# Gardlin/PCR-CG

Measured on AMD Instinct MI355X. Metric: fragment-pairs/s KPFCNN+GCN fwd, 30k-pt pairs, higher is better.
Workload: dtype f32

## Files before the change

include/pcrcg.h:

```cpp
#ifndef PCRCG_H
#define PCRCG_H

#include <stddef.h>
#include <stdint.h>

#ifdef __cplusplus
extern "C" {
#endif

#define PCRCG_OK 0
#define PCRCG_EBADARG (-1)
#define PCRCG_EWORKSPACE (-2)
#define PCRCG_ELAUNCH (-3)
#define PCRCG_ECAPACITY (-4)

#define PCRCG_KPOINTS 15

const char* pcrcg_last_error(void);
#define PCRCG_ABI_VERSION 4
int pcrcg_abi_version(void);

int pcrcg_debug_set(const char* spec);
int pcrcg_debug_release(void);

// ... 47 lines not shown
                         const void* forest, int cloud0, float radius, const int* rows, int nrows, const int* count,
                         int max_count, int cols, int64_t* idx, int* status, void* stream);
int pcrcg_radius_reorder_jobs(const pcrcg_reorder_job* jobs, int njobs, const float* sup, int ns, int nb,
                              const void* forest, int* status, void* stream);

size_t pcrcg_kpconv_ws_bytes(int ns);
int pcrcg_kpconv_aggregate(const float* q_pts, int nq, const float* s_pts, int ns, const int64_t* idx,
                           int h, int ld_idx, const float* x, int cin, const float* kp, float extent,
                           float* wf, float* inv_n, void* ws, size_t ws_bytes, void* stream);
int pcrcg_kpconv_aggregate_bf16(const float* q_pts, int nq, const float* s_pts, int ns, const int64_t* idx, int h,
                                int ld_idx, const float* x, int cin, const float* kp, float extent, void* x_bf16,
                                void* wf_bf16, float* inv_n, void* ws, size_t ws_bytes, void* stream);

void pcrcg_profile_kpconv(int enable);
int pcrcg_profile_kpconv_read(float* ms, int* nq, int* h, int* cin, int* cout, int* kind, int cap);

int pcrcg_gemm_f32(const float* a, int lda, const float* b, int ldb, int trans_b, float* c, int ldc, int m,
                   int n, int k, const float* row_scale, const float* bias, void* stream);
size_t pcrcg_gemm_colstats_bytes(int m, int n);
int pcrcg_gemm_f32_colstats(const float* a, int lda, const float* b, int ldb, int trans_b, float* c, int ldc,
                            int m, int n, int k, const float* row_scale, const float* bias, void* colstats,
                            size_t colstats_bytes, int* h_chunks, void* stream);
int pcrcg_gemm_bf16a_f32_colstats(const void* a_bf16, int lda, const float* b, int ldb, float* c, int ldc, int m, int n,
                                  int k, const float* row_scale, const float* bias, void* colstats,
                                  size_t colstats_bytes, int* h_chunks, void* stream);

int pcrcg_gemm_f32_fused(const float* a, int lda, const int64_t* idx, int ld_idx, int ns, const float* zero_row,
                         const void* a_sums, double a_count, float a_eps, float a_slope, const float* b, int ldb,
                         const float* bias, float* c, int ldc, int m, int n, int k, int accumulate, void* stream);

void pcrcg_gemm_set_mode(int mode);
int pcrcg_gemm_get_mode(void);
int pcrcg_gemm_redo_counts(unsigned long long* out2, int reset);
void pcrcg_thread_shares_gpu(int on);

int pcrcg_gather_max(const float* x, int ns, int c, const int64_t* idx, int nq, int h, int ld_idx,
                     float* out, void* stream);
int pcrcg_gather_first(const float* x, int ns, int c, const int64_t* idx, int nq, int ld_idx, float* out,
                       int ld_out, void* stream);
size_t pcrcg_instnorm_ws_bytes(int c);
int pcrcg_instnorm_stats_from_partials(const void* partials, int chunks, int c, double count, float eps,
                                       float* stats, void* stream);
int pcrcg_instnorm_stats(const float* x, int n, int c, int ldx, float eps, float* stats, void* ws,
                         size_t ws_bytes, void* stream);
int pcrcg_instnorm_apply(const float* x, int n, int c, int ldx, const float* stats, const float* res,
                         int ldr, const float* res_stats, float slope, float* y, int ldy, void* stream);
int pcrcg_instnorm_colsums(const float* x, int n, int c, int ldx, void* sums, void* stream);
int pcrcg_instnorm_apply_sums(const float* x, int n, int c, int ldx, const void* sums, double count, float eps,
                              const float* res, int ldr, const void* res_sums, float slope, float* y, int ldy,
                              void* stream);

int pcrcg_fill2d(float* dst, int ld, int rows, int cols, float value, void* stream);
int pcrcg_inject_image_features(const float* fmap, int c, int h, int w, const float* valid, const int64_t* inds2d,
                                const int64_t* inds3d, int n, long row_offset, long n_rows, float* x, int ldx,
                                void* stream);

typedef struct pcrcg_image_frame {
    const float* fmap;
    const float* depth;
    const float* valid;
    float world2camera[16];
    float intrinsics[16];
    float thresh;
    int h, w;
    int depth_h, depth_w;
    int target;
// ... 190 lines not shown
```

pcrcg_amd/_lib.py:

```python
import ctypes
import os

_HERE = os.path.dirname(os.path.abspath(__file__))
LIB_PATH = os.path.join(_HERE, "libpcrcg_hip.so")


def lib_identity():
    import hashlib
    with open(LIB_PATH, "rb") as f:
        return LIB_PATH, hashlib.sha256(f.read()).hexdigest()[:16]

ABI_VERSION = 4

c_int, c_float, c_void_p, c_size_t = ctypes.c_int, ctypes.c_float, ctypes.c_void_p, ctypes.c_size_t

SIGNATURES = {
    "pcrcg_last_error": (ctypes.c_char_p, []),
    "pcrcg_abi_version": (c_int, []),
    "pcrcg_debug_set": (c_int, [ctypes.c_char_p]),
    "pcrcg_check_status": (c_int, [c_void_p, c_void_p]),
    "pcrcg_grid_subsample_ws_bytes": (c_size_t, [c_int, c_int]),
    "pcrcg_grid_subsample_batch": (c_int, [c_void_p, c_int, c_void_p, c_int, c_float, c_int, c_void_p, c_void_p,
                                           c_void_p, c_void_p, c_size_t, c_void_p]),
    "pcrcg_umap_order_ws_bytes": (c_size_t, [c_int]),
# ... 7 lines not shown
    "pcrcg_radius_query_groups": (c_int, [c_void_p, c_int, c_void_p, c_int, c_void_p, c_int, c_int, c_float, c_void_p, c_int,
                                          c_void_p, c_void_p, c_void_p, c_void_p, c_void_p, c_void_p, c_void_p]),
    "pcrcg_radius_query_cells": (c_int, [c_void_p, c_void_p, c_int, c_void_p, c_void_p, c_int, c_void_p, c_int, c_int, c_float,
                                         c_int, c_void_p, c_void_p, c_void_p, c_void_p, c_void_p, c_void_p, c_void_p]),
    "pcrcg_kdforest_ws_bytes": (c_size_t, [c_int, c_int]),
    "pcrcg_kdforest_build": (c_int, [c_void_p, c_int, c_void_p, c_int, c_void_p, c_size_t, c_void_p]),
    "pcrcg_radius_reorder": (c_int, [c_void_p, c_int, c_void_p, c_int, c_void_p, c_int, c_int, c_void_p, c_int,
                                     c_float, c_void_p, c_int, c_void_p, c_int, c_int, c_void_p, c_void_p, c_void_p]),
    "pcrcg_radius_reorder_jobs": (c_int, [c_void_p, c_int, c_void_p, c_int, c_int, c_void_p, c_void_p, c_void_p]),
    "pcrcg_radius_neighbors_ws_bytes": (c_size_t, [c_int, c_int]),
    "pcrcg_radius_neighbors_batch": (c_int, [c_void_p, c_int, c_void_p, c_int, c_void_p, c_void_p, c_int, c_float,
                                             c_int, c_void_p, c_void_p, c_void_p, c_void_p, c_void_p, c_size_t,
                                             c_void_p]),
    "pcrcg_kpconv_ws_bytes": (c_size_t, [c_int]),
    "pcrcg_kpconv_aggregate": (c_int, [c_void_p, c_int, c_void_p, c_int, c_void_p, c_int, c_int, c_void_p, c_int,
                                       c_void_p, c_float, c_void_p, c_void_p, c_void_p, c_size_t, c_void_p]),
    "pcrcg_kpconv_aggregate_bf16": (c_int, [c_void_p, c_int, c_void_p, c_int, c_void_p, c_int, c_int, c_void_p, c_int,
                                            c_void_p, c_float, c_void_p, c_void_p, c_void_p, c_void_p, c_size_t,
                                            c_void_p]),
    "pcrcg_profile_kpconv": (None, [c_int]),
    "pcrcg_profile_kpconv_read": (c_int, [c_void_p, c_void_p, c_void_p, c_void_p, c_void_p, c_void_p, c_int]),
    "pcrcg_gemm_f32": (c_int, [c_void_p, c_int, c_void_p, c_int, c_int, c_void_p, c_int, c_int, c_int, c_int,
                               c_void_p, c_void_p, c_void_p]),
    "pcrcg_gemm_colstats_bytes": (c_size_t, [c_int, c_int]),
    "pcrcg_gemm_f32_colstats": (c_int, [c_void_p, c_int, c_void_p, c_int, c_int, c_void_p, c_int, c_int, c_int, c_int,
                                        c_void_p, c_void_p, c_void_p, c_size_t, c_void_p, c_void_p]),
    "pcrcg_gemm_bf16a_f32_colstats": (c_int, [c_void_p, c_int, c_void_p, c_int, c_void_p, c_int, c_int, c_int, c_int,
                                              c_void_p, c_void_p, c_void_p, c_size_t, c_void_p, c_void_p]),
    "pcrcg_gemm_f32_fused": (c_int, [c_void_p, c_int, c_void_p, c_int, c_int, c_void_p, c_void_p, ctypes.c_double, c_float,
                                     c_float, c_void_p, c_int, c_void_p, c_void_p, c_int, c_int, c_int, c_int, c_int, c_void_p]),
    "pcrcg_gemm_set_mode": (None, [c_int]),
    "pcrcg_gemm_get_mode": (c_int, []),
    "pcrcg_gemm_redo_counts": (c_int, [c_void_p, c_int]),
    "pcrcg_instnorm_stats_from_partials": (c_int, [c_void_p, c_int, c_int, ctypes.c_double, c_float, c_void_p,
                                                   c_void_p]),
    "pcrcg_gather_max": (c_int, [c_void_p, c_int, c_int, c_void_p, c_int, c_int, c_int, c_void_p, c_void_p]),
    "pcrcg_gather_first": (c_int, [c_void_p, c_int, c_int, c_void_p, c_int, c_int, c_void_p, c_int, c_void_p]),
    "pcrcg_instnorm_ws_bytes": (c_size_t, [c_int]),
    "pcrcg_instnorm_stats": (c_int, [c_void_p, c_int, c_int, c_int, c_float, c_void_p, c_void_p, c_size_t, c_void_p]),
    "pcrcg_instnorm_apply": (c_int, [c_void_p, c_int, c_int, c_int, c_void_p, c_void_p, c_int, c_void_p, c_float,
                                     c_void_p, c_int, c_void_p]),
    "pcrcg_instnorm_colsums": (c_int, [c_void_p, c_int, c_int, c_int, c_void_p, c_void_p]),
    "pcrcg_instnorm_apply_sums": (c_int, [c_void_p, c_int, c_int, c_int, c_void_p, ctypes.c_double, c_float, c_void_p, c_int,
                                          c_void_p, c_float, c_void_p, c_int, c_void_p]),
    "pcrcg_fill2d": (c_int, [c_void_p, c_int, c_int, c_int, c_float, c_void_p]),
    "pcrcg_inject_image_features": (c_int, [c_void_p, c_int, c_int, c_int, c_void_p, c_void_p, c_void_p, c_int, ctypes.c_long,
                                            ctypes.c_long, c_void_p, c_int, c_void_p]),
    "pcrcg_project_depth_ws_bytes": (c_size_t, [c_int]),
    "pcrcg_project_depth": (c_int, [c_void_p, c_int, c_void_p, c_int, c_int, c_void_p, c_void_p, c_float, c_void_p, c_void_p,
                                    c_void_p, c_void_p, c_size_t, c_void_p]),
    "pcrcg_inject_frames": (c_int, [c_void_p, ctypes.c_long, ctypes.c_long, c_void_p, c_int, c_int, c_void_p, c_int, c_void_p]),
    "pcrcg_superglue_valid_maps": (c_int, [c_void_p, c_int, c_void_p, c_int, c_void_p, c_void_p, c_int, c_int, c_int, c_void_p,
                                           c_void_p, c_void_p]),
    "pcrcg_knn": (c_int, [c_void_p, c_int, c_int, c_void_p, c_void_p]),
    "pcrcg_edgeconv_ws_bytes": (c_size_t, [c_int]),
    "pcrcg_edgeconv_reduce": (c_int, [c_void_p, c_int, c_void_p, c_int, c_void_p, c_int, c_int, c_int, c_float,
                                      c_void_p, c_int, c_void_p, c_void_p, c_size_t, c_void_p]),
    "pcrcg_edgeconv_reduce_sums": (c_int, [c_void_p, c_int, c_void_p, c_int, c_void_p, c_int, c_int, c_int, c_void_p, c_int,
                                           c_void_p, c_void_p]),
    "pcrcg_softmax_rows": (c_int, [c_void_p, c_int, c_int, c_int, c_float, c_void_p]),
    "pcrcg_attention_supported": (c_int, [c_int]),
    "pcrcg_attention": (c_int, [c_void_p, c_int, c_void_p, c_int, c_void_p, c_int, c_void_p, c_int, c_int, c_int, c_int,
                                c_int, c_float, c_void_p]),
    "pcrcg_softmax_matvec": (c_int, [c_void_p, c_int, c_int, c_int, c_float, c_void_p, c_int, c_void_p, c_int, c_void_p]),
    "pcrcg_copy2d": (c_int, [c_void_p, c_int, c_void_p, c_int, c_int, c_int, c_void_p]),
    "pcrcg_add": (c_int, [c_void_p, c_void_p, c_void_p, ctypes.c_long, c_void_p]),
# ... 117 lines not shown
```

pcrcg_amd/csrc/common.h:

```cpp
#pragma once
#include <hip/hip_runtime.h>

#include <cstdarg>
#include <cstdint>
#include <cstdio>
#include <mutex>

#include "pcrcg.h"

namespace pcrcg {

void set_error(const char* fmt, ...);

inline hipStream_t as_stream(void* s) { return reinterpret_cast<hipStream_t>(s); }

struct Carver {
    char* base;
    size_t cap;
    size_t off = 0;
    Carver(void* ws, size_t bytes) : base(static_cast<char*>(ws)), cap(bytes) {}
    template <typename T>
    T* take(size_t count) {
        size_t bytes = (count * sizeof(T) + 255) & ~size_t(255);
        T* p = reinterpret_cast<T*>(base + off);
// ... 87 lines not shown
int gather_max_multi(const GatherJob* jobs, int count, int c, hipStream_t st);
int heads_multi(const float* const* x, const int* rows, int count, int ld, int fd, float* const* feats, float* const* s_ov,
                float* const* s_sal, hipStream_t st);
int copy2d_multi(const float* const* src, float* const* dst, const int* rows, int count, int ld_src, int ld_dst, int cols,
                 hipStream_t st);
int instnorm_colsums_multi(const float* const* x, double* const* sums, const int* n, int count, int c, int ldx, hipStream_t st);

struct EdgeCloud {
    const float* ctr; const float* nbr; const int* idx; float* emax; double* sums; int n, k;
};
bool edgeconv_rows_ok(const EdgeCloud* cl, int count, int ld_ctr, int ld_nbr, int ld_emax, int c);
int edgeconv_rows_multi(const EdgeCloud* cl, int count, int ld_ctr, int ld_nbr, int ld_emax, int c, bool atomic, int* nchunks_out,
                        hipStream_t st);

struct AttnCloud { const float* q; const float* k; const float* v; float* out; int n, ms; };
bool attention_mfma_ok(const AttnCloud* cl, int count, int ldq, int ldk, int ldv, int d);
int attention_mfma_multi(const AttnCloud* cl, int count, int ldq, int ldk, int ldv, int ldo, int heads, int d, float scale,
                         hipStream_t st);
bool attention_bwd_mfma_ok(int n, int ms, int d, int ldq, int ldk, int ldv, int ld_do);
int attention_bwd_mfma(const float* q, int ldq, const float* k, int ldk, const float* v, int ldv, const float* o, int ldo,
                       const float* d_o, int ld_do, float* dq, int ld_dq, float* dk, int ld_dk, float* dv, int ld_dv, int n, int ms,
                       int heads, int d, float scale, hipStream_t st);

struct DebugOpts {
    int stat_sums = 1;
    int stat_sums_rows = 1 << 30;
    int att_mfma = 1;
    int radius_blocks = 0;
    int kd_blocks = 0;
    int att_tq = 16;
    int kd_spin_limit = 0;
    int gemm_log = 0;
    int x6_tile = -1, x6_splitk = 0, x6_t1 = 1, x6_t2 = 1, x6_order = -1, x6_big = 0, x6_h2 = 1;
    int train_side_stream = 1;
    int gemm_tile = -1, gemm_splitk = 0, gemm_split_target = 768;
    int deterministic = 0;
    int bwd_mfma = 1;
};
const DebugOpts& debug_opts();

struct KpProfScope {
    hipStream_t st;
    hipEvent_t a, b;
    int nq, h, cin, cout, kind;
    bool on;
    KpProfScope(hipStream_t s, int nq, int h, int cin, int cout, int kind);
    ~KpProfScope();
};

}

#define PCRCG_CHECK_ARG(cond)                                                        \
    do {                                                                             \
        if (!(cond)) {                                                               \
            pcrcg::set_error("%s: bad argument: %s", __func__, #cond);               \
            return PCRCG_EBADARG;                                                    \
        }                                                                            \
    } while (0)

#define PCRCG_CHECK_WS(carver)                                                                     \
    do {                                                                                           \
        if (!(carver).ok()) {                                                                      \
            pcrcg::set_error("%s: workspace too small (%zu needed, %zu given)", __func__,          \
                             (carver).off, (carver).cap);                                          \
            return PCRCG_EWORKSPACE;                                                               \
        }                                                                                          \
// ... 36 lines not shown
```

pcrcg_amd/csrc/gemm.hip:

```cpp
#include <cstdlib>

#include <atomic>

#include "common.h"
#include "pcrcg_train.h"

namespace pcrcg {
namespace {

typedef float f32x16 __attribute__((ext_vector_type(16)));
template <int BM, int BN, bool TRANS_A, bool TRANS_B, int BK>
constexpr int stage_floats() {
    return (TRANS_A ? BK * (BM + 4) : BM * (BK + 4)) + (TRANS_B ? BN * (BK + 4) : BK * (BN + 4));
}

template <int BM, int BN, int WAVES_M, int WAVES_N, bool TRANS_A, bool TRANS_B, int BK>
__global__ void __launch_bounds__(256) k_gemm_f32(const float* __restrict__ A, int lda, const float* __restrict__ B,
                                                   int ldb, float* __restrict__ C, int ldc, int M, int N, int Kdim,
                                                   const float* __restrict__ row_scale, const float* __restrict__ bias,
                                                   int k_per_split, int vec_a, int vec_b, int atomic_out,
                                                   double* __restrict__ colp, int colp_chunks) {
    static_assert(WAVES_M * WAVES_N == 4, "4 wavefronts per block");
    constexpr int WM = BM / WAVES_M, WN = BN / WAVES_N;
    constexpr int TM = WM / 32, TN = WN / 32;
// ... 272 lines not shown
                                                          k_per_split, vec_a, vec_b, atomic_out, colp, colp_chunks);
    return launch_one<BM, BN, WAVES_M, WAVES_N, false, false, BK>(grid, st, a, lda, b, ldb, c, ldc, m, n, k, row_scale, bias,
                                                       k_per_split, vec_a, vec_b, atomic_out, colp, colp_chunks);
}

}
}

namespace pcrcg {
int gemm_x6_dispatch(const float* a, int lda, const float* b, int ldb, float* c, int ldc, int m, int n, int k,
                     const float* row_scale, const float* bias, void* colstats, size_t colstats_bytes, int* h_chunks,
                     hipStream_t st, bool a_bf16, bool c_zeroed, int a_kmajor = 0, int b_kmajor = 0,
                     bool colstats_sums = false, const GemmExtra* ex = nullptr, const GemmGroup* grp = nullptr);
int gemm_x6_splits(int m, int n, int k, long m_total = 0);
}

using namespace pcrcg;

static std::atomic<int> g_gemm_mode{-1};
static int gemm_mode() {
    int mode = g_gemm_mode.load(std::memory_order_relaxed);
    if (mode < 0) {
        const char* e = getenv("PCRCG_GEMM_MODE");
        int want = e ? (atoi(e) != 0) : 1, expect = -1;
        g_gemm_mode.compare_exchange_strong(expect, want, std::memory_order_relaxed);
        mode = g_gemm_mode.load(std::memory_order_relaxed);
    }
    return mode;
}
extern "C" void pcrcg_gemm_set_mode(int mode) { g_gemm_mode.store(mode != 0, std::memory_order_relaxed); }
extern "C" void pcrcg_thread_shares_gpu(int on) { gemm_x6_set_shared(on); }
namespace pcrcg { int gemm_x6_redo_counts(unsigned long long* out, int reset); }
extern "C" int pcrcg_gemm_redo_counts(unsigned long long* out2, int reset) { return gemm_x6_redo_counts(out2, reset); }
extern "C" int pcrcg_gemm_get_mode(void) { return gemm_mode(); }

static int gemm_dispatch(const float* a, int lda, int trans_a, const float* b, int ldb, int trans_b, float* c, int ldc,
                         int m, int n, int k, const float* row_scale, const float* bias, void* colstats,
                         size_t colstats_bytes, int* h_chunks, void* stream, bool c_zeroed = false,
                         bool colstats_sums = false);

namespace pcrcg {
bool gemm_bt_accumulates(int m, int n, int k, long m_total) { return gemm_mode() == 1 && gemm_x6_splits(m, n, k, m_total) > 1; }
bool gemm_colstats_sums_ok() { return gemm_mode() == 1; }
bool gemm_extra_ok() { return gemm_mode() == 1; }
int gemm_bt_extra(const float* a, int lda, const float* b, int ldb, float* c, int ldc, int m, int n, int k, hipStream_t st,
                  bool c_zeroed, const GemmExtra& ex, const float* bias, void* colstats, size_t colstats_bytes, int* h_chunks,
                  bool colstats_sums) {
    if (h_chunks) *h_chunks = 0;
    PCRCG_CHECK_ARG(m >= 0 && n >= 0 && k >= 1 && lda >= k && ldb >= k && ldc >= n);
    if (m == 0 || n == 0) return PCRCG_OK;
    PCRCG_CHECK_ARG(a && b && c && gemm_mode() == 1);
    return gemm_x6_dispatch(a, lda, b, ldb, c, ldc, m, n, k, nullptr, bias, colstats, colstats_bytes, h_chunks, st, false,
                            c_zeroed, 0, 0, colstats_sums, &ex);
}
bool gemm_pair_ok() { return gemm_mode() == 1; }
int gemm_bt_colstats_pair(const float* a, int lda, const float* b, int ldb, float* c, int ldc, int m, int n, int k,
                          const float* row_scale, const float* bias, void* colstats, size_t colstats_bytes, int* h_chunks,
                          hipStream_t st, bool c_zeroed, bool colstats_sums, const GemmGroup* pair) {
    if (!pair || pair->n == 0)
        return gemm_dispatch(a, lda, 0, b, ldb, 1, c, ldc, m, n, k, row_scale, bias, colstats, colstats_bytes, h_chunks, st,
                             c_zeroed, colstats_sums);
    if (h_chunks) *h_chunks = 0;
    PCRCG_CHECK_ARG(m >= 1 && n >= 1 && k >= 1 && lda >= k && ldb >= k && ldc >= n);
    PCRCG_CHECK_ARG(a && b && c && gemm_mode() == 1);
    return gemm_x6_dispatch(a, lda, b, ldb, c, ldc, m, n, k, row_scale, bias, colstats, colstats_bytes, h_chunks, st, false,
                            c_zeroed, 0, 0, colstats_sums, nullptr, pair);
// ... 184 lines not shown
```

pcrcg_amd/csrc/gemm_x6.hip:

```cpp
#include <cstdlib>
#include <map>
#include <mutex>
#include <type_traits>

#include <hip/hip_ext.h>

#include "common.h"
#include "pcrcg_train.h"

namespace pcrcg {
namespace {

typedef float f32x16 __attribute__((ext_vector_type(16)));
typedef __bf16 bf16x8 __attribute__((ext_vector_type(8)));
typedef unsigned int u32x4 __attribute__((ext_vector_type(4)));

typedef float f32x4 __attribute__((ext_vector_type(4)));
typedef float f32x2 __attribute__((ext_vector_type(2)));
typedef _Float16 f16x2 __attribute__((ext_vector_type(2)));
typedef _Float16 f16x8 __attribute__((ext_vector_type(8)));

constexpr int BK = 32;

__device__ unsigned long long g_x6_redo[2];

constexpr int kGroupExtra = 3;
struct GemmPairArgs {
    int extra = 0;
    int off[kGroupExtra] = {0, 0, 0}, m[kGroupExtra] = {0, 0, 0};
    const float* a[kGroupExtra] = {nullptr, nullptr, nullptr};
    float* c[kGroupExtra] = {nullptr, nullptr, nullptr};
    const float* rs[kGroupExtra] = {nullptr, nullptr, nullptr};
// ... 662 lines not shown
        double* const red = reinterpret_cast<double*>(smem);
        __syncthreads();
#pragma unroll
        for (int j = 0; j < TN; ++j) {
            const double s = ds[j] + __shfl_xor(ds[j], 32, 64), q2 = dq[j] + __shfl_xor(dq[j], 32, 64);
            if (wm == 1 && half == 0) {
                red[2 * (wn * WN + j * 32 + l31)] = s;
                red[2 * (wn * WN + j * 32 + l31) + 1] = q2;
            }
        }
        __syncthreads();
#pragma unroll
        for (int j = 0; j < TN; ++j) {
            const double s = ds[j] + __shfl_xor(ds[j], 32, 64), q2 = dq[j] + __shfl_xor(dq[j], 32, 64);
            const int gn = n0 + wn * WN + j * 32 + l31;
            if (wm == 0 && half == 0 && gn < N) {
                unsafeAtomicAdd(&colp[gn], s + red[2 * (wn * WN + j * 32 + l31)]);
                unsafeAtomicAdd(&colp[(long)N + gn], q2 + red[2 * (wn * WN + j * 32 + l31) + 1]);
            }
        }
    } else if (colp) {
        const int chunk = tile_y * WAVES_M + wm;
#pragma unroll
        for (int j = 0; j < TN; ++j) {
            const double s = ds[j] + __shfl_xor(ds[j], 32, 64), q2 = dq[j] + __shfl_xor(dq[j], 32, 64);
            const int gn = n0 + wn * WN + j * 32 + l31;
            if (half == 0 && gn < N) {
                colp[(long)gn * colp_chunks + chunk] = s;
                colp[((long)N + gn) * colp_chunks + chunk] = q2;
            }
        }
    }
}

thread_local long g_split_stride = 0;
thread_local bool g_det_pass = false;
struct DetBuf { float* p = nullptr; size_t n = 0; };
std::mutex g_det_mu;
std::map<hipStream_t, DetBuf> g_det_bufs;
float* det_partials(hipStream_t st, size_t floats) {
    std::lock_guard<std::mutex> g(g_det_mu);
    DetBuf& b = g_det_bufs[st];
    if (b.n < floats) {
        if (hipStreamSynchronize(st) != hipSuccess) return nullptr;
        if (b.p) (void)hipFree(b.p);
        b.p = nullptr;
        b.n = 0;
        const size_t want = floats + floats / 4;
        if (hipMalloc(&b.p, want * sizeof(float)) != hipSuccess) { b.p = nullptr; return nullptr; }
        b.n = want;
    }
    return b.p;
}

__global__ void __launch_bounds__(256) k_split_reduce(const float* __restrict__ part, long stride, int splits, float* __restrict__ c,
                                                      int ldc, int m, int n, int accumulate) {
    const long t = (long)blockIdx.x * 256 + threadIdx.x;
    if (t >= (long)m * n) return;
    const long r = t / n;
    const int col = (int)(t - r * n);
    float sum = part[t];
    for (int s = 1; s < splits; ++s) sum += part[(long)s * stride + t];
    float* dst = c + r * ldc + col;
    *dst = accumulate ? *dst + sum : sum;
}

template <int BM, int BN, int MINB, int ATERMS, int ALAY, int BLAY, int ANORM = 0, int KNOCK = 0, int H2 = 0>
int launch_x6(dim3 grid, hipStream_t st, const float* a, int lda, const float* b, int ldb, float* c, int ldc, int m, int n,
              int k, const float* row_scale, const float* bias, int k_per_split, int vec_a, int vec_b, int atomic_out,
              double* colp, int colp_chunks, const long long* a_idx = nullptr, int a_idx_ld = 0, int a_ns = 0,
              const float* a_zero = nullptr, const double* a_sums = nullptr, double a_count = 0.0, float a_eps = 0.f,
              float a_slope = 1.f, GemmPairArgs pr = GemmPairArgs(), float h2_sa = 1.f, float h2_sb = 1.f) {
    TileMap tm;
    tm.split_stride = g_split_stride;
    tm.gx = (int)grid.x;
    tm.gy = (int)grid.y;
    tm.gs = (int)grid.z;
    tm.order = x6_tile_order(tm.gx, tm.gy, tm.gs, BM, BN, k_per_split);
    const size_t lds = lds_bytes<BM, BN>() + (ANORM ? 2 * sizeof(float) * (size_t)(((k_per_split + BK - 1) / BK) * BK) : 0) + (H2 ? 16 : 0);
    auto kern = k_gemm_x6<BM, BN, MINB, ATERMS, ALAY, BLAY, ANORM, KNOCK, H2>;
    PCRCG_GRANT_LDS(kern);
    int m_all = m;
    for (int e = 0; e < pr.extra; ++e) m_all += pr.m[e];
    KpProfScope prof(st, m_all, n, k, (ATERMS == 1 || H2) ? 3 : 6, 3);
    hipExtLaunchKernelGGL(kern, dim3(tm.gx * tm.gy * tm.gs), dim3(x6_threads<BM, BN>()), lds, st, prof.a, prof.b, 0, a, lda, b, ldb, c, ldc, m, n,
                          k, row_scale, bias, k_per_split, vec_a, vec_b, atomic_out, colp, colp_chunks, a_idx, a_idx_ld, a_ns,
                          a_zero, a_sums, a_count, a_eps, a_slope, pr, tm, h2_sa, h2_sb);
    PCRCG_CHECK_LAUNCH();
    return PCRCG_OK;
}


}

static thread_local int g_x6_shared = 0;
bool gemm_x6_shared() { return g_x6_shared > 0; }
void gemm_x6_set_shared(int on) { g_x6_shared = on ? 1 : 0; }

struct X6Plan { int pick, bm, bn, gx, gy, splits, k_per_split; };
static X6Plan x6_plan_for(int pick, int m, int n, int k, bool reduce_rows) {
    static const int tiles[4][2] = {{128, 128}, {128, 64}, {64, 128}, {64, 64}};
    X6Plan p;
    p.pick = pick;
    p.bm = tiles[p.pick][0];
    p.bn = tiles[p.pick][1];
    p.gx = (n + p.bn - 1) / p.bn;
    p.gy = (m + p.bm - 1) / p.bm;
    int splits = 1;
    const int ktiles = (k + BK - 1) / BK;
    const int max_splits = reduce_rows ? 128 : 32;
    int t1 = 200, t2 = 1024;
    if (gemm_x6_shared() && !reduce_rows) { t1 = debug_opts().x6_t1; t2 = debug_opts().x6_t2; }
    while ((long)p.gx * p.gy * splits < t1 && k / (2 * splits) >= 256 && splits < max_splits) splits *= 2;
    while ((long)p.gx * p.gy * splits < t2 && k / splits > 1024 && splits < max_splits) splits *= 2;
    if (debug_opts().x6_splitk > 0) splits = debug_opts().x6_splitk;
    p.k_per_split = ((ktiles + splits - 1) / splits) * BK;
    if (p.k_per_split < BK) p.k_per_split = BK;
    p.splits = k > 0 ? (k + p.k_per_split - 1) / p.k_per_split : 1;
    if (p.splits < 1) p.splits = 1;
    return p;
}
static X6Plan x6_plan(int m, int n, int k, bool kmajor = false, bool reduce_rows = false, long m_total = 0) {
    int pick = debug_opts().x6_tile;
    if (kmajor) return x6_plan_for(3, m, n, k, reduce_rows);
    if (pick >= 0 && pick <= 3) return x6_plan_for(pick, m, n, k, reduce_rows);
    if (n >= 128 && debug_opts().x6_big) {
        const X6Plan big = x6_plan_for(0, m, n, k, reduce_rows);
        const long rows = m_total > m ? m_total : m;
        if ((long)big.gx * ((rows + 127) / 128) * big.splits >= 240) return big;
    }
    return x6_plan_for((n <= 64 && m >= 32768) ? 1 : 3, m, n, k, reduce_rows);
}

int gemm_x6_redo_counts(unsigned long long* out, int reset) {
    if (out) PCRCG_CHECK_HIP(hipMemcpyFromSymbol(out, HIP_SYMBOL(g_x6_redo), sizeof(unsigned long long) * 2));
    if (reset) {
        const unsigned long long z[2] = {0ull, 0ull};
        PCRCG_CHECK_HIP(hipMemcpyToSymbol(HIP_SYMBOL(g_x6_redo), z, sizeof(z)));
    }
    return PCRCG_OK;
}

int gemm_x6_splits(int m, int n, int k, long m_total) { return (m > 0 && n > 0) ? x6_plan(m, n, k, false, false, m_total).splits : 1; }

void gemm_x6_release_det() {
    std::lock_guard<std::mutex> g(g_det_mu);
    for (auto& kv : g_det_bufs)
        if (kv.second.p) (void)hipFree(kv.second.p);
    g_det_bufs.clear();
}

int gemm_x6_dispatch(const float* a, int lda, const float* b, int ldb, float* c, int ldc, int m, int n, int k,
                     const float* row_scale, const float* bias, void* colstats, size_t colstats_bytes, int* h_chunks,
                     hipStream_t st, bool a_bf16, bool c_zeroed, int a_kmajor, int b_kmajor, bool colstats_sums,
                     const GemmExtra* ex, const GemmGroup* grp) {
    const int vec_a = (a_bf16 || a_kmajor) ? 1 : (lda % 4 == 0) && ((reinterpret_cast<uintptr_t>(a) & 15) == 0);
    const int vec_b = b_kmajor ? 1 : (ldb % 4 == 0) && ((reinterpret_cast<uintptr_t>(b) & 15) == 0);
    if (a_kmajor && !b_kmajor) { set_error("gemm_x6: A^T * B^T is not built"); return PCRCG_EBADARG; }
    int m_plan = m;
    const int n_extra = grp ? grp->n : 0;
    if (n_extra < 0 || n_extra > kGroupExtra) { set_error("gemm_x6: at most %d further products per launch", kGroupExtra); return PCRCG_EBADARG; }
    for (int e = 0; e < n_extra; ++e) {
        if (grp->p[e].m <= 0 || !grp->p[e].a || !grp->p[e].c) { set_error("gemm_x6: empty product in a group"); return PCRCG_EBADARG; }
        m_plan = grp->p[e].m > m_plan ? grp->p[e].m : m_plan;
    }
    long m_total = m;
    for (int e = 0; e < n_extra; ++e) m_total += grp->p[e].m;
    const bool lifted = ex && ex->grad_operand && debug_opts().x6_h2 != 0 && !a_bf16;
    const X6Plan plan = x6_plan(m_plan, n, k, a_kmajor || b_kmajor || (ex && ex->a_sums) || lifted, a_kmajor != 0, m_total);
    const int pick = plan.pick, BM = plan.bm, BN = plan.bn, gx = plan.gx, splits = plan.splits;
    const int gy0 = (m + BM - 1) / BM;
    int gy = gy0, gye[kGroupExtra] = {0, 0, 0};
    for (int e = 0; e < n_extra; ++e) { gye[e] = (grp->p[e].m + BM - 1) / BM; gy += gye[e]; }
    if (n_extra && (a_kmajor || b_kmajor)) { set_error("gemm_x6: grouped launches are built for the A * B^T form"); return PCRCG_EBADARG; }
    const int k_per_split = plan.k_per_split;
// ... 28 lines not shown
                grp2.p[e].h_chunks = nullptr;
                row += (size_t)grp->p[e].m;
            }
        }
        g_det_pass = true;
        g_split_stride = (long)(rows_all * (size_t)n);
        const int rc = gemm_x6_dispatch(a, lda, b, ldb, part, n, m, n, k, row_scale, bias, nullptr, 0, nullptr, st, a_bf16, true,
                                        a_kmajor, b_kmajor, false, ex ? &ex2 : nullptr, grp ? &grp2 : nullptr);
        g_det_pass = false;
        g_split_stride = 0;
        if (rc != PCRCG_OK) return rc;
        row = 0;
        for (int e = -1; e < n_extra; ++e) {
            const int me = e < 0 ? m : grp->p[e].m;
            float* ce = e < 0 ? c : grp->p[e].c;
            const long total = (long)me * n;
            hipLaunchKernelGGL(k_split_reduce, dim3((unsigned)((total + 255) / 256)), dim3(256), 0, st, part + row * (size_t)n,
                               (long)(rows_all * (size_t)n), splits, ce, ldc, me, n, accumulate ? 1 : 0);
            row += (size_t)me;
        }
        PCRCG_CHECK_LAUNCH();
        return PCRCG_OK;
    }
    const int atomic_out = g_det_pass ? 0 : (splits > 1 || accumulate);
    if (splits > 1 && !c_zeroed && !accumulate) {
        if (ldc == n) PCRCG_CHECK_HIP(hipMemsetAsync(c, 0, (size_t)m * n * sizeof(float), st));
        else PCRCG_CHECK_HIP(hipMemset2DAsync(c, (size_t)ldc * sizeof(float), 0, (size_t)n * sizeof(float), m, st));
    }
    for (int e = 0; e < n_extra; ++e)
        if (splits > 1 && !grp->p[e].c_zeroed && !accumulate) {
            if (ldc == n) PCRCG_CHECK_HIP(hipMemsetAsync(grp->p[e].c, 0, (size_t)grp->p[e].m * n * sizeof(float), st));
            else PCRCG_CHECK_HIP(hipMemset2DAsync(grp->p[e].c, (size_t)ldc * sizeof(float), 0, (size_t)n * sizeof(float), grp->p[e].m, st));
        }
    dim3 grid(gx, gy, splits);
    const bool log_shapes = debug_opts().gemm_log != 0;
    if (log_shapes)
        fprintf(stderr, "pcrcg_gemm_x6 m=%d n=%d k=%d lda=%d ldb=%d ldc=%d tile=%dx%d grid=%dx%dx%d rs=%d bias=%d stats=%d\n", m,
                n, k, lda, ldb, ldc, BM, BN, gx, gy, splits, row_scale != nullptr, bias != nullptr, colstats != nullptr);
    double* colp = nullptr;
    int colp_chunks = 0;
    if (colstats && h_chunks && !atomic_out && colstats_sums) {
        if (2 * (size_t)n * sizeof(double) <= colstats_bytes) {
            colp = static_cast<double*>(colstats);
            colp_chunks = -1;
            *h_chunks = -1;
        }
    } else if (colstats && h_chunks && !atomic_out) {
        colp_chunks = gy0 * 2;
        if (carve_bytes(2 * (size_t)n * colp_chunks, sizeof(double)) <= colstats_bytes) {
            colp = static_cast<double*>(colstats);
            *h_chunks = colp_chunks;
        } else {
            colp_chunks = 0;
        }
    }
    GemmPairArgs pa;
    pa.extra = n_extra;
    int row_off = gy0 * BM;
    for (int e = 0; e < n_extra; ++e) {
        const GemmPair& q = grp->p[e];
        pa.off[e] = row_off;
        row_off += gye[e] * BM;
        pa.m[e] = q.m;
        pa.a[e] = q.a;
        pa.c[e] = q.c;
        pa.rs[e] = q.row_scale;
// ... 79 lines not shown
```

pcrcg_amd/csrc/scan.hip:

```cpp
#include <cstring>

#include <atomic>
#include <mutex>

#include "common.h"

namespace pcrcg {

static thread_local char g_err[512] = "";

void set_error(const char* fmt, ...) {
    va_list ap;
    va_start(ap, fmt);
    vsnprintf(g_err, sizeof(g_err), fmt, ap);
    va_end(ap);
}

namespace {

constexpr int kScanThreads = 256;
constexpr int kScanItems = 8;
constexpr int kScanTile = kScanThreads * kScanItems;

__device__ __forceinline__ int wave_inclusive_scan(int v, int lane) {
// ... 145 lines not shown
int exclusive_scan_i32(const int* in, int* out, int n, int* total, void* ws, hipStream_t stream) {
    if (n <= 0) {
        if (total) hipLaunchKernelGGL(zero_int, dim3(1), dim3(1), 0, stream, total);
        PCRCG_CHECK_LAUNCH();
        return PCRCG_OK;
    }
    const int nt = (n + kScanTile - 1) / kScanTile;
    if (nt == 1) {
        hipLaunchKernelGGL(scan_apply, dim3(1), dim3(kScanThreads), 0, stream, in, out, n,
                           (const int*)nullptr, total);
        PCRCG_CHECK_LAUNCH();
        return PCRCG_OK;
    }
    if (n <= kOneTiles * kOneThreads * kScanItems && (reinterpret_cast<uintptr_t>(in) & 15) == 0 &&
        (reinterpret_cast<uintptr_t>(out) & 15) == 0) {
        hipLaunchKernelGGL(scan_one_block, dim3(1), dim3(kOneThreads), 0, stream, in, out, n, total);
        PCRCG_CHECK_LAUNCH();
        return PCRCG_OK;
    }
    int* partial = static_cast<int*>(ws);
    hipLaunchKernelGGL(scan_tile_sums, dim3(nt), dim3(kScanThreads), 0, stream, in, n, partial);
    hipLaunchKernelGGL(scan_partials, dim3(1), dim3(kScanThreads), 0, stream, partial, nt, total);
    hipLaunchKernelGGL(scan_apply, dim3(nt), dim3(kScanThreads), 0, stream, in, out, n,
                       (const int*)partial, (int*)nullptr);
    PCRCG_CHECK_LAUNCH();
    return PCRCG_OK;
}

namespace {
struct DebugName { const char* name; int DebugOpts::*field; };
const DebugName kDebugNames[] = {
    {"stat_sums", &DebugOpts::stat_sums}, {"stat_sums_rows", &DebugOpts::stat_sums_rows}, {"att_mfma", &DebugOpts::att_mfma},
    {"radius_blocks", &DebugOpts::radius_blocks}, {"kd_blocks", &DebugOpts::kd_blocks}, {"att_tq", &DebugOpts::att_tq},
    {"kd_spin_limit", &DebugOpts::kd_spin_limit}, {"gemm_log", &DebugOpts::gemm_log}, {"x6_tile", &DebugOpts::x6_tile}, {"x6_order", &DebugOpts::x6_order}, {"x6_big", &DebugOpts::x6_big}, {"x6_h2", &DebugOpts::x6_h2}, {"train_side_stream", &DebugOpts::train_side_stream},
    {"x6_splitk", &DebugOpts::x6_splitk}, {"x6_t1", &DebugOpts::x6_t1}, {"x6_t2", &DebugOpts::x6_t2},
    {"gemm_tile", &DebugOpts::gemm_tile}, {"gemm_splitk", &DebugOpts::gemm_splitk},
    {"gemm_split_target", &DebugOpts::gemm_split_target}, {"deterministic", &DebugOpts::deterministic},
    {"bwd_mfma", &DebugOpts::bwd_mfma}};
std::atomic<const DebugOpts*> g_debug{nullptr};
std::atomic<const DebugOpts*> g_debug_env{nullptr};
std::once_flag g_debug_once;
std::mutex g_debug_set_lock;
const DebugOpts kDebugDefaults{};

bool debug_parse(const char* spec, const DebugOpts* base) {
    DebugOpts d = *base;
    const char* p = spec;
    while (p && *p) {
        const char* end = strchr(p, ',');
        const size_t len = end ? (size_t)(end - p) : strlen(p);
        const char* eq = static_cast<const char*>(memchr(p, '=', len));
        bool ok = false;
        if (eq) {
            for (const DebugName& n : kDebugNames)
                if (strlen(n.name) == (size_t)(eq - p) && strncmp(n.name, p, (size_t)(eq - p)) == 0) {
                    d.*(n.field) = atoi(eq + 1);
                    ok = true;
                }
        }
        if (!ok && len > 0) {
            set_error("pcrcg_debug_set: unknown or malformed item '%.*s'", (int)len, p);
            return false;
        }
        p = end ? end + 1 : nullptr;
    }
    if (d.deterministic) {
        d.stat_sums = 0;
// ... 57 lines not shown
```

Measured before the change: 598.0.

## Add B-resident row-walking GEMM kernel for small-K tall matrices

New measurement: 601.8, median of 3. About the same (+0.6%).

```diff
diff --git a/include/pcrcg.h b/include/pcrcg.h
--- a/include/pcrcg.h
+++ b/include/pcrcg.h
@@ -103,6 +103,7 @@
 void pcrcg_gemm_set_mode(int mode);
 int pcrcg_gemm_get_mode(void);
 int pcrcg_gemm_redo_counts(unsigned long long* out2, int reset);
+int pcrcg_gemm_walk_launches(unsigned long long* out, int reset);
 void pcrcg_thread_shares_gpu(int on);
 
 int pcrcg_gather_max(const float* x, int ns, int c, const int64_t* idx, int nq, int h, int ld_idx,
diff --git a/pcrcg_amd/_lib.py b/pcrcg_amd/_lib.py
--- a/pcrcg_amd/_lib.py
+++ b/pcrcg_amd/_lib.py
@@ -63,6 +63,7 @@
     "pcrcg_gemm_set_mode": (None, [c_int]),
     "pcrcg_gemm_get_mode": (c_int, []),
     "pcrcg_gemm_redo_counts": (c_int, [c_void_p, c_int]),
+    "pcrcg_gemm_walk_launches": (c_int, [c_void_p, c_int]),
     "pcrcg_instnorm_stats_from_partials": (c_int, [c_void_p, c_int, c_int, ctypes.c_double, c_float, c_void_p,
                                                    c_void_p]),
     "pcrcg_gather_max": (c_int, [c_void_p, c_int, c_int, c_void_p, c_int, c_int, c_int, c_void_p, c_void_p]),
diff --git a/pcrcg_amd/csrc/common.h b/pcrcg_amd/csrc/common.h
--- a/pcrcg_amd/csrc/common.h
+++ b/pcrcg_amd/csrc/common.h
@@ -143,6 +143,7 @@
     int kd_spin_limit = 0;
     int gemm_log = 0;
     int x6_tile = -1, x6_splitk = 0, x6_t1 = 1, x6_t2 = 1, x6_order = -1, x6_big = 0, x6_h2 = 1;
+    int x6_walk = 1;
     int train_side_stream = 1;
     int gemm_tile = -1, gemm_splitk = 0, gemm_split_target = 768;
     int deterministic = 0;
diff --git a/pcrcg_amd/csrc/gemm.hip b/pcrcg_amd/csrc/gemm.hip
--- a/pcrcg_amd/csrc/gemm.hip
+++ b/pcrcg_amd/csrc/gemm.hip
@@ -328,6 +328,8 @@
 extern "C" void pcrcg_thread_shares_gpu(int on) { gemm_x6_set_shared(on); }
 namespace pcrcg { int gemm_x6_redo_counts(unsigned long long* out, int reset); }
 extern "C" int pcrcg_gemm_redo_counts(unsigned long long* out2, int reset) { return gemm_x6_redo_counts(out2, reset); }
+namespace pcrcg { int gemm_x6_walk_launches(unsigned long long* out, int reset); }
+extern "C" int pcrcg_gemm_walk_launches(unsigned long long* out, int reset) { return gemm_x6_walk_launches(out, reset); }
 extern "C" int pcrcg_gemm_get_mode(void) { return gemm_mode(); }
 
 static int gemm_dispatch(const float* a, int lda, int trans_a, const float* b, int ldb, int trans_b, float* c, int ldc,
diff --git a/pcrcg_amd/csrc/gemm_x6.hip b/pcrcg_amd/csrc/gemm_x6.hip
--- a/pcrcg_amd/csrc/gemm_x6.hip
+++ b/pcrcg_amd/csrc/gemm_x6.hip
@@ -1,3 +1,4 @@
+#include <atomic>
 #include <cstdlib>
 #include <map>
 #include <mutex>
@@ -726,6 +727,263 @@
         }
     }
 }
+
+constexpr int kWalkBM = 64, kWalkBN = 64, kWalkMaxK = 256;
+static size_t walk_lds_bytes(int k, bool anorm) {
+    return (size_t)(k / BK) * 2 * kWalkBN * ROWB + 2 * kWalkBM * ROWB + (2 * kWalkBM + kWalkBN + 4) * 4 + (anorm ? 2 * sizeof(float) * (size_t)k : 0);
+}
+template <int ANORM>
+__global__ void __launch_bounds__(256, 4) k_gemm_x6_walk(const float* __restrict__ A, int lda, const float* __restrict__ B, int ldb,
+                                                         float* __restrict__ C, int ldc, int M, int N, int Kdim,
+                                                         const float* __restrict__ row_scale, const float* __restrict__ bias,
+                                                         double* __restrict__ colp, int colp_chunks,
+                                                         const double* __restrict__ a_sums, double a_count, float a_eps,
+                                                         float a_slope, GemmPairArgs pr, int gx, int nchunk, int rt) {
+    constexpr int BM = kWalkBM, BN = kWalkBN, NT = 256;
+    constexpr int A_PLANE = BM * ROWB, B_PLANE = BN * ROWB;
+    extern __shared__ __attribute__((aligned(16))) unsigned char smem[];
+    const int nk = Kdim / BK;
+    unsigned char* const Bres = smem;
+    unsigned char* const As = smem + (size_t)nk * 2 * B_PLANE;
+    unsigned* const s_seen = reinterpret_cast<unsigned*>(As + 2 * A_PLANE);
+    unsigned* const s_seenb = s_seen + 2 * BM;
+    int* const s_flag = reinterpret_cast<int*>(s_seenb + BN);
+    float* const s_mean = reinterpret_cast<float*>(s_flag + 4);
+    float* const s_rstd = s_mean + (ANORM ? Kdim : 0);
+
+    const int tid = threadIdx.x, lane = tid & 63, wave = __builtin_amdgcn_readfirstlane((int)(threadIdx.x >> 6));
+    const int wm = wave >> 1, wn = wave & 1, half = lane >> 5, l31 = lane & 31;
+    const int ntile = gx * nchunk, lin = blockIdx.x;
+    const int xq = ntile >> 3, xr = ntile & 7, xcd = lin & 7, slot = lin >> 3;
+    const int tile = (xcd < xr ? xcd * (xq + 1) : xr * (xq + 1) + (xcd - xr) * xq) + slot;
+    const int tile_x = tile % gx;
+    int chunk = tile / gx;
+    if (pr.extra > 0 && chunk >= pr.off[0]) {
+        int e = 0;
+        if (pr.extra > 1 && chunk >= pr.off[1]) e = 1;
+        if (pr.extra > 2 && chunk >= pr.off[2]) e = 2;
+        chunk -= pr.off[e];
+        M = pr.m[e];
+        A = pr.a[e];
+        C = pr.c[e];
+        row_scale = pr.rs[e];
+        colp = pr.colp[e];
+        colp_chunks = pr.colp_chunks[e];
+        a_sums = pr.a_sums[e];
+        a_count = pr.a_count[e];
+    }
+    const int n0 = tile_x * BN;
+    const int t0 = chunk * rt;
+    const int ntl = min(rt, (M + BM - 1) / BM - t0);
+
+    for (int i = tid; i < 2 * BM + BN + 4; i += NT) s_seen[i] = 0u;
+    if constexpr (ANORM) {
+        for (int kk = tid; kk < Kdim; kk += NT) {
+            const double mu = a_sums[kk] / a_count;
+            double var = a_sums[(long)Kdim + kk] / a_count - mu * mu;
+            if (var < 0.0) var = 0.0;
+            s_mean[kk] = (float)mu;
+            s_rstd[kk] = (float)(1.0 / sqrt(var + (double)a_eps));
+        }
+    }
+    __syncthreads();
+    auto store_h = [&](unsigned char* base, int plane_bytes, int row, int kg, const Item<0>& src) {
+        unsigned q1[4], q2[4];
+#pragma unroll
+        for (int j = 0; j < 4; ++j) split2h(src.get(2 * j), src.get(2 * j + 1), q1[j], q2[j]);
+        const u32x4 p1 = {q1[0], q1[1], q1[2], q1[3]}, p2 = {q2[0], q2[1], q2[2], q2[3]};
+        unsigned char* d = base + row * ROWB + kg * 16;
+        *reinterpret_cast<u32x4*>(d) = p1;
+        *reinterpret_cast<u32x4*>(d + plane_bytes) = p2;
+    };
+    auto largest = [&](const Item<0>& src, float seen) {
+#pragma unroll
+        for (int j = 0; j < 4; ++j) seen = fmaxf(fmaxf(fabsf(src.get(2 * j)), fabsf(src.get(2 * j + 1))), seen);
+        return seen;
+    };
+    for (int e = tid; e < BN * 4 * nk; e += NT) {
+        const int row = e / (4 * nk), kga = e % (4 * nk), c = kga >> 2, kg = kga & 3;
+        const float* p = B + (long)min(n0 + row, N - 1) * ldb + kga * 8;
+        Item<0> q;
+        q.v[0] = *reinterpret_cast<const f32x4*>(p);
+        q.v[1] = *reinterpret_cast<const f32x4*>(p + 4);
+        const float seen = largest(q, 0.f);
+        if (seen > 0.f) atomicMax(&s_seenb[row], __float_as_uint(seen));
+        store_h(Bres + (size_t)c * 2 * B_PLANE, B_PLANE, row, kg, q);
+    }
+    __syncthreads();
+    if (tid < BN) {
+        const unsigned v = s_seenb[tid];
+        if (v != 0u && v < 0x38800000u) atomicOr(&s_flag[2], 1);
+        if (v >= 0x477ff000u) atomicOr(&s_flag[2], 2);
+    }
+    __syncthreads();
+    const int bflag = s_flag[2];
+
+    const int a_row = tid >> 2, a_kg = tid & 3;
+    auto row_ptr = [&](int t) { return A + (long)min((t0 + t) * BM + a_row, M - 1) * lda + a_kg * 8; };
+    auto issue = [&](Item<0>& q, const float* rowp, int c) {
+        gload16(q.v[0], rowp + c * BK);
+        gload16(q.v[1], rowp + c * BK + 4);
+    };
+    float seen_a = 0.f;
+    auto consume = [&](Item<0>& q, int c) {
+        vm_wait<2>();
+        q.hold();
+        if constexpr (ANORM) {
+#pragma unroll
+            for (int j = 0; j < 8; ++j) {
+                const int kk = c * BK + a_kg * 8 + j;
+                const float v = (q.get(j) - s_mean[kk]) * s_rstd[kk];
+                q.set(j, v >= 0.f ? v : v * a_slope);
+            }
+        }
+        seen_a = largest(q, seen_a);
+        __builtin_amdgcn_sched_barrier(0);
+        __syncthreads();
+        store_h(As, A_PLANE, a_row, a_kg, q);
+    };
+    f32x16 acc, acc_lo;
+    auto multiply = [&](int c) {
+        const unsigned char* const Bc = Bres + (size_t)c * 2 * B_PLANE;
+#pragma unroll
+        for (int cc = 0; cc < BK / 16; ++cc) {
+            f16x8 a[2], b[2];
+#pragma unroll
+            for (int p = 0; p < 2; ++p) {
+                a[p] = __builtin_bit_cast(f16x8, *reinterpret_cast<const u32x4*>(As + p * A_PLANE + (wm * 32 + l31) * ROWB + (cc * 2 + half) * 16));
+                b[p] = __builtin_bit_cast(f16x8, *reinterpret_cast<const u32x4*>(Bc + p * B_PLANE + (wn * 32 + l31) * ROWB + (cc * 2 + half) * 16));
+            }
+            acc_lo = __builtin_amdgcn_mfma_f32_32x32x16_f16(a[1], b[0], acc_lo, 0, 0, 0);
+            acc = __builtin_amdgcn_mfma_f32_32x32x16_f16(a[0], b[0], acc, 0, 0, 0);
+            acc_lo = __builtin_amdgcn_mfma_f32_32x32x16_f16(a[0], b[1], acc_lo, 0, 0, 0);
+        }
+    };
+
+    const int gn = n0 + wn * 32 + l31;
+    const float bv = bias ? bias[min(gn, N - 1)] : 0.0f;
+    double run_s = 0.0, run_q = 0.0;
+
+    Item<0> ra[2];
+    const float* rp = row_ptr(0);
+    issue(ra[0], rp, 0);
+    issue(ra[1], rp, 1);
+    for (int t = 0; t < ntl; ++t) {
+        const float* const rp_next = row_ptr(min(t + 1, ntl - 1));
+#pragma unroll
+        for (int r = 0; r < 16; ++r) { acc[r] = 0.0f; acc_lo[r] = 0.0f; }
+        seen_a = 0.f;
+        for (int c = 0; c + 2 < nk; c += 2) {
+            consume(ra[0], c);
+            issue(ra[0], rp, c + 2);
+            __syncthreads();
+            multiply(c);
+            consume(ra[1], c + 1);
+            issue(ra[1], rp, c + 3);
+            __syncthreads();
+            multiply(c + 1);
+        }
+        consume(ra[0], nk - 2);
+        issue(ra[0], rp_next, 0);
+        __syncthreads();
+        multiply(nk - 2);
+        consume(ra[1], nk - 1);
+        issue(ra[1], rp_next, 1);
+        __syncthreads();
+        multiply(nk - 1);
+        rp = rp_next;
+
+        const int par = t & 1;
+        const int m0 = (t0 + t) * BM;
+        bool bad = false;
+#pragma unroll
+        for (int r = 0; r < 16; ++r) bad = bad || !(fabsf(acc[r]) <= 3.0e38f) || !(fabsf(acc_lo[r]) <= 3.0e38f);
+        if (bad) atomicOr(&s_flag[par], 2);
+        if (seen_a > 0.f) atomicMax(&s_seen[par * BM + a_row], __float_as_uint(seen_a));
+        if (tid < BM) s_seen[(par ^ 1) * BM + tid] = 0u;
+        if (tid == 0) s_flag[par ^ 1] = 0;
+        __syncthreads();
+        if (tid < BM) {
+            const unsigned v = s_seen[par * BM + tid];
+            if (v != 0u && v < 0x38800000u) atomicOr(&s_flag[par], 1);
+        }
+        __syncthreads();
+        const int flag = s_flag[par] | bflag;
+        if (flag != 0) {
+            if (tid == 0) atomicAdd(&g_x6_redo[(flag & 2) ? 0 : 1], 1ull);
+            const float* const brow = B + (long)min(gn, N - 1) * ldb;
+#pragma unroll 1
+            for (int r = 0; r < 16; ++r) {
+                const int gm = m0 + wm * 32 + (r & 3) + 8 * (r >> 2) + 4 * half;
+                const float* const arow = A + (long)min(gm, M - 1) * lda;
+                double sum = 0.0;
+                for (int kk = 0; kk < Kdim; kk += 4) {
+                    f32x4 av = *reinterpret_cast<const f32x4*>(arow + kk);
+                    const f32x4 bw = *reinterpret_cast<const f32x4*>(brow + kk);
+#pragma unroll
+                    for (int j = 0; j < 4; ++j) {
+                        if constexpr (ANORM) {
+                            const float v = (av[j] - s_mean[kk + j]) * s_rstd[kk + j];
+                            av[j] = v >= 0.f ? v : v * a_slope;
+                        }
+                        sum += (double)av[j] * (double)bw[j];
+                    }
+                }
+#pragma unroll
+                for (int rr = 0; rr < 16; ++rr) acc[rr] = rr == r ? (float)sum : acc[rr];
+            }
+        } else {
+#pragma unroll
+            for (int r = 0; r < 16; ++r) acc[r] = acc[r] + acc_lo[r] * (1.0f / kH2Scale);
+        }
+
+        float cs = 0.f, cq = 0.f, piv = 0.f;
+        int cnt = 0;
+#pragma unroll
+        for (int r = 0; r < 16; ++r) {
+            const int gm = m0 + wm * 32 + (r & 3) + 8 * (r >> 2) + 4 * half;
+            const float rsv = row_scale ? row_scale[min(gm, M - 1)] : 1.0f;
+            const float v = acc[r] * rsv + bv;
+            if (r == 0) piv = v;
+            if (gm < M && gn < N) {
+                C[(long)gm * ldc + gn] = v;
+                const float d = v - piv;
+                cs += d;
+                cq += d * d;
+            }
+            cnt += gm < M ? 1 : 0;
+        }
+        if (colp) {
+            const double p = cnt ? (double)piv : 0.0, s1 = (double)cs;
+            run_s += s1 + (double)cnt * p;
+            run_q += (double)cq + p * (2.0 * s1 + (double)cnt * p);
+        }
+    }
+    vm_wait<0>();
+
+    if (colp) {
+        double* const red = reinterpret_cast<double*>(As);
+        const double s = run_s + __shfl_xor(run_s, 32, 64), q2 = run_q + __shfl_xor(run_q, 32, 64);
+        __syncthreads();
+        if (wm == 1 && half == 0) {
+            red[2 * (wn * 32 + l31)] = s;
+            red[2 * (wn * 32 + l31) + 1] = q2;
+        }
+        __syncthreads();
+        if (wm == 0 && half == 0 && gn < N) {
+            const double ts = s + red[2 * (wn * 32 + l31)], tq = q2 + red[2 * (wn * 32 + l31) + 1];
+            if (colp_chunks < 0) {
+                unsafeAtomicAdd(&colp[gn], ts);
+                unsafeAtomicAdd(&colp[(long)N + gn], tq);
+            } else {
+                colp[(long)gn * colp_chunks + chunk] = ts;
+                colp[((long)N + gn) * colp_chunks + chunk] = tq;
+            }
+        }
+    }
+}
+
+std::atomic<unsigned long long> g_walk_launches{0};
 
 thread_local long g_split_stride = 0;
 thread_local bool g_det_pass = false;
@@ -784,6 +1042,21 @@
     return PCRCG_OK;
 }
 
+template <int ANORM>
+int launch_walk(hipStream_t st, const float* a, int lda, const float* b, int ldb, float* c, int ldc, int m, int n, int k,
+                const float* row_scale, const float* bias, double* colp, int colp_chunks, const double* a_sums, double a_count,
+                float a_eps, float a_slope, const GemmPairArgs& pr, int gx, int nchunk, int rt) {
+    auto kern = k_gemm_x6_walk<ANORM>;
+    PCRCG_GRANT_LDS(kern);
+    int m_all = m;
+    for (int e = 0; e < pr.extra; ++e) m_all += pr.m[e];
+    KpProfScope prof(st, m_all, n, k, 3, 3);
+    hipExtLaunchKernelGGL(kern, dim3(gx * nchunk), dim3(256), walk_lds_bytes(k, ANORM != 0), st, prof.a, prof.b, 0, a, lda, b, ldb, c,
+                          ldc, m, n, k, row_scale, bias, colp, colp_chunks, a_sums, a_count, a_eps, a_slope, pr, gx, nchunk, rt);
+    PCRCG_CHECK_LAUNCH();
+    g_walk_launches.fetch_add(1, std::memory_order_relaxed);
+    return PCRCG_OK;
+}
 
 }
 
@@ -835,6 +1108,12 @@
     return PCRCG_OK;
 }
 
+int gemm_x6_walk_launches(unsigned long long* out, int reset) {
+    const unsigned long long v = reset ? g_walk_launches.exchange(0, std::memory_order_relaxed) : g_walk_launches.load(std::memory_order_relaxed);
+    if (out) *out = v;
+    return PCRCG_OK;
+}
+
 int gemm_x6_splits(int m, int n, int k, long m_total) { return (m > 0 && n > 0) ? x6_plan(m, n, k, false, false, m_total).splits : 1; }
 
 void gemm_x6_release_det() {
@@ -929,6 +1208,61 @@
             if (ldc == n) PCRCG_CHECK_HIP(hipMemsetAsync(grp->p[e].c, 0, (size_t)grp->p[e].m * n * sizeof(float), st));
             else PCRCG_CHECK_HIP(hipMemset2DAsync(grp->p[e].c, (size_t)ldc * sizeof(float), 0, (size_t)n * sizeof(float), grp->p[e].m, st));
         }
+    const int walk_opt = debug_opts().x6_walk;
+    if (walk_opt != 0 && debug_opts().x6_h2 != 0 && !a_bf16 && !a_kmajor && !b_kmajor && !(ex && ex->grad_operand) && !gather &&
+        !accumulate && splits == 1 && !g_det_pass && vec_a && vec_b && k >= 64 && k <= kWalkMaxK && k % 64 == 0) {
+        const int gxw = (n + kWalkBN - 1) / kWalkBN;
+        int gyw[1 + kGroupExtra] = {(m + kWalkBM - 1) / kWalkBM, 0, 0, 0};
+        long tiles = (long)gxw * gyw[0];
+        bool ok = true;
+        for (int e = 0; e < n_extra; ++e) {
+            gyw[e + 1] = (grp->p[e].m + kWalkBM - 1) / kWalkBM;
+            tiles += (long)gxw * gyw[e + 1];
+            ok = ok && (reinterpret_cast<uintptr_t>(grp->p[e].a) & 15) == 0 && !grp->p[e].a_idx;
+        }
+        if (walk_opt == 1 && (k != 64 || tiles < 2048)) ok = false;
+        if (ok) {
+            int rt = (int)((tiles + 1023) / 1024);
+            rt = rt < 4 ? 4 : rt > 16 ? 16 : rt;
+            GemmPairArgs pw;
+            pw.extra = n_extra;
+            const int chunks0 = (gyw[0] + rt - 1) / rt;
+            int nchunk = chunks0;
+            double* colp = nullptr;
+            int colp_chunks = 0;
+            if (colstats && h_chunks && colstats_sums) {
+                if (2 * (size_t)n * sizeof(double) <= colstats_bytes) { colp = static_cast<double*>(colstats); colp_chunks = -1; }
+            } else if (colstats && h_chunks) {
+                if (carve_bytes(2 * (size_t)n * chunks0, sizeof(double)) <= colstats_bytes) { colp = static_cast<double*>(colstats); colp_chunks = chunks0; }
+            }
+            if (colp) *h_chunks = colp_chunks;
+            for (int e = 0; e < n_extra; ++e) {
+                const GemmPair& q = grp->p[e];
+                const int ce = (gyw[e + 1] + rt - 1) / rt;
+                pw.off[e] = nchunk;
+                nchunk += ce;
+                pw.m[e] = q.m;
+                pw.a[e] = q.a;
+                pw.c[e] = q.c;
+                pw.rs[e] = q.row_scale;
+                pw.a_sums[e] = q.a_sums;
+                pw.a_count[e] = q.a_count;
+                if (q.h_chunks) *q.h_chunks = 0;
+                if (colp && q.colstats && q.h_chunks && (colp_chunks < 0 || carve_bytes(2 * (size_t)n * ce, sizeof(double)) <= colstats_bytes)) {
+                    pw.colp[e] = static_cast<double*>(q.colstats);
+                    pw.colp_chunks[e] = colp_chunks < 0 ? -1 : ce;
+                    *q.h_chunks = pw.colp_chunks[e];
+                }
+            }
+            if (debug_opts().gemm_log != 0)
+                fprintf(stderr, "pcrcg_gemm_x6 m=%d n=%d k=%d walk grid=%dx%d rt=%d norm=%d stats=%d\n", m, n, k, gxw, nchunk, rt, (int)anorm, colp_chunks);
+            if (anorm)
+                return launch_walk<1>(st, a, lda, b, ldb, c, ldc, m, n, k, row_scale, bias, colp, colp_chunks, ex->a_sums, ex->a_count,
+                                      ex->a_eps, ex->a_slope, pw, gxw, nchunk, rt);
+            return launch_walk<0>(st, a, lda, b, ldb, c, ldc, m, n, k, row_scale, bias, colp, colp_chunks, nullptr, 0.0, 0.f, 1.f, pw,
+                                  gxw, nchunk, rt);
+        }
+    }
     dim3 grid(gx, gy, splits);
     const bool log_shapes = debug_opts().gemm_log != 0;
     if (log_shapes)
diff --git a/pcrcg_amd/csrc/scan.hip b/pcrcg_amd/csrc/scan.hip
--- a/pcrcg_amd/csrc/scan.hip
+++ b/pcrcg_amd/csrc/scan.hip
@@ -201,7 +201,7 @@
 const DebugName kDebugNames[] = {
     {"stat_sums", &DebugOpts::stat_sums}, {"stat_sums_rows", &DebugOpts::stat_sums_rows}, {"att_mfma", &DebugOpts::att_mfma},
     {"radius_blocks", &DebugOpts::radius_blocks}, {"kd_blocks", &DebugOpts::kd_blocks}, {"att_tq", &DebugOpts::att_tq},
-    {"kd_spin_limit", &DebugOpts::kd_spin_limit}, {"gemm_log", &DebugOpts::gemm_log}, {"x6_tile", &DebugOpts::x6_tile}, {"x6_order", &DebugOpts::x6_order}, {"x6_big", &DebugOpts::x6_big}, {"x6_h2", &DebugOpts::x6_h2}, {"train_side_stream", &DebugOpts::train_side_stream},
+    {"kd_spin_limit", &DebugOpts::kd_spin_limit}, {"gemm_log", &DebugOpts::gemm_log}, {"x6_tile", &DebugOpts::x6_tile}, {"x6_order", &DebugOpts::x6_order}, {"x6_big", &DebugOpts::x6_big}, {"x6_h2", &DebugOpts::x6_h2}, {"x6_walk", &DebugOpts::x6_walk}, {"train_side_stream", &DebugOpts::train_side_stream},
     {"x6_splitk", &DebugOpts::x6_splitk}, {"x6_t1", &DebugOpts::x6_t1}, {"x6_t2", &DebugOpts::x6_t2},
     {"gemm_tile", &DebugOpts::gemm_tile}, {"gemm_splitk", &DebugOpts::gemm_splitk},
     {"gemm_split_target", &DebugOpts::gemm_split_target}, {"deterministic", &DebugOpts::deterministic},
```
